# victorkich/ManyTor

Hardware: AMD Instinct MI355X
Metric: env-steps/sec (whole node), 1M parallel 4-DoF arms, random actions (higher is better)
Workload: dtype f32

## Files before the change

### manytor_amd/csrc/engine.hip

```cpp
#include <hip/hip_runtime.h>

#include <algorithm>
#include <cmath>
#include <cstdio>
#include <cstdlib>
#include <cstring>
#include <mutex>
#include <new>
#include <iterator>
#include <string>
#include <utility>
#include <vector>

#include "engine_internal.h"
#include "kernels.h"

using namespace mt;

namespace {
thread_local std::string g_last_error;
}

namespace mt {
int fail(mt_handle h, int code, const std::string& msg) {
// ... 72 lines not shown

struct BlockCap {
  int64_t from, below;
  int blocks;
};
struct DispatchPolicy {
  int64_t step_split4_max = 49152, step_split2_max = 65536;
  int64_t prefetch_other_max = 131072;
  int64_t fused_split4_max = 32768, fused_split2_max = 131072;
  int64_t reset_split_max = 65536;
  int64_t graph_max = 131072;
  int64_t chains_min = 163840, chains_max = 3145728;
  int64_t chain_split4_max = 16384, chain_split2_max = 49152, chain_prefetch_other_max = 131072;
  int64_t flat_from = 393216;
  BlockCap block_caps[3] = {{147456, 229376, 3}, {229376, 458752, 4}, {458752, 589824, 5}};
  int64_t multi_step_max = 262144;
  int multi_step_k = 5;
  bool fold_reset_into_chains = false;
  int max_recurrence_rotations = 12;
  bool rederive_goals_ref4 = true;
  bool rederive_goals_dh7 = false;
  int rederive_goals_chains = 1;
  int64_t rederive_goals_max_envs = 3145728;
  int64_t ld_pad_above = 16384;
  int ld_pad_floats = 256;
};
static const DispatchPolicy kPolicy{};

static int step_blocks_per_cu(const mt_engine* h, int64_t n_launch) {
  if (h->blocks_per_cu_override >= 0) return h->blocks_per_cu_override;
  if (n_launch >= h->n) return 0;
  for (const BlockCap& c : kPolicy.block_caps)
    if (n_launch >= c.from && n_launch < c.below) return c.blocks;
  return 0;
}
static size_t lds_pad_for_blocks(int blocks_per_cu, size_t static_lds) {
  if (blocks_per_cu <= 0) return 0;
  const size_t per_block = (size_t)163840 / (size_t)blocks_per_cu - 1024;
  return per_block > static_lds ? std::min<size_t>(per_block, 65536) - static_lds : 0;
}

int64_t chain_span(const mt_engine* h, int chains) {
  const int64_t per = (h->n + chains - 1) / chains;
  return (per + 255) / 256 * 256;
}

static bool env_int(const char* name, long long* v) {
  const char* e = std::getenv(name);
  if (!e || !*e) return false;
  *v = std::atoll(e);
  return true;
}

static void choose_dispatch(mt_handle h) {
  const mt_config* cfg = &h->cfg;
  const DispatchPolicy& P = kPolicy;
  const int64_t n = cfg->n_envs;
  long long v = 0;
  h->overrides.clear();
  auto seen = [&](const char* name) { h->overrides += (h->overrides.empty() ? "" : ",") + std::string(name) + "=" + std::to_string(v); };

  h->trig = (cfg->flags & MT_FLAG_HW_TRIG) ? 2 : ((cfg->flags & MT_FLAG_DIRECT_TRIG) ? 1 : 0);
  if (cfg->flags & MT_FLAG_ABLATE_LOOP) h->trig = (cfg->flags & MT_FLAG_ABLATE_OBS) ? 4 : 3;
  else if (cfg->flags & MT_FLAG_ABLATE_OBS) h->trig = 5;
  const bool long_route = h->trig == 0 && (cfg->substeps - 1) / 2 > P.max_recurrence_rotations;
  if (long_route) h->trig = 1;
  h->lds_table = (cfg->flags & MT_FLAG_DH_IN_LDS) != 0 && !long_route;
  h->custom_frames = !(h->args.dh.fo == h->D - 2 && h->args.dh.fe == h->D - 1);
  h->static_kind = ((cfg->flags & (MT_FLAG_NO_SPECIALIZE | MT_FLAG_DH_IN_LDS)) || h->custom_frames) ? 0 : match_static(h->args.dh, h->D);

  int forced_lanes = 0, forced_prefetch = -1;
  if (env_int("MT_SPLIT", &v)) {
    forced_lanes = (v == 2 || v == 4) ? (int)v : 1;
    seen("MT_SPLIT");
  }
  if (env_int("MT_PREFETCH", &v)) {
    forced_prefetch = v != 0;
    seen("MT_PREFETCH");
  }
  h->reset_split = n <= P.reset_split_max;
  if (env_int("MT_RESET_SPLIT", &v)) {
    h->reset_split = v != 0;
    seen("MT_RESET_SPLIT");
  }
  h->graph_mode = -1;
  h->graph_max = P.graph_max;
  if (env_int("MT_GRAPH", &v)) {
    h->graph_mode = v != 0 ? 1 : 0;
    seen("MT_GRAPH");
  }
  h->flat_from = P.flat_from;
  if (env_int("MT_FLAT_FROM", &v)) {
    h->flat_from = std::max<long long>(0, v);
    seen("MT_FLAT_FROM");
  }
  h->blocks_per_cu_override = -1;
  if (env_int("MT_BLOCKS_PER_CU", &v)) {
    const int c = (int)std::max<long long>(0, std::min<long long>(8, v));
    h->blocks_per_cu_override = (c == 1 || c == 2) ? 3 : c;
    seen("MT_BLOCKS_PER_CU");
  }
  h->trig_steps = h->static_kind != 0;
  if (env_int("MT_TRIG_TABLE", &v)) {
    h->trig_steps = v != 0 && h->static_kind != 0;
    seen("MT_TRIG_TABLE");
  }
// ... 10 lines not shown
  if (env_int("MT_LAZY_CHAINS", &v)) {
    h->lazy_chains = v != 0;
    seen("MT_LAZY_CHAINS");
  }

  h->multi_k = (n <= P.multi_step_max) ? P.multi_step_k : 1;
  if (env_int("MT_ROLLOUT_K", &v)) {
    h->multi_k = (int)std::max<long long>(1, std::min<long long>(64, v));
    seen("MT_ROLLOUT_K");
  }
  h->defer_reset = true;
  if (env_int("MT_DEFER_RESET", &v)) {
    h->defer_reset = v != 0;
    seen("MT_DEFER_RESET");
  }
  h->defer_reset_chained = P.fold_reset_into_chains;
  if (env_int("MT_DEFER_RESET_CHAINS", &v)) {
    h->defer_reset_chained = v != 0;
    seen("MT_DEFER_RESET_CHAINS");
  }
  h->gather_throttle = true;
  if (env_int("MT_GATHER_THROTTLE", &v)) {
    h->gather_throttle = v != 0;
    seen("MT_GATHER_THROTTLE");
  }
  h->snap_in_rollout = true;
  if (env_int("MT_ROLLOUT_SNAP", &v)) {
    h->snap_in_rollout = v != 0;
    seen("MT_ROLLOUT_SNAP");
  }
  h->rollout_early = true;
  if (env_int("MT_ROLLOUT_EARLY", &v)) {
    h->rollout_early = v != 0;
    seen("MT_ROLLOUT_EARLY");
  }

  h->tape_prefetch = false;
  if (env_int("MT_TAPE_PREFETCH", &v)) {
    h->tape_prefetch = v != 0;
    seen("MT_TAPE_PREFETCH");
  }
  h->tape_nt_loads = false;
  if (env_int("MT_TAPE_NT", &v)) {
    h->tape_nt_loads = v != 0;
    seen("MT_TAPE_NT");
  }

  h->ground_compact = true;
  if (env_int("MT_GROUND_COMPACT", &v)) {
    h->ground_compact = v != 0;
    seen("MT_GROUND_COMPACT");
  }

  h->goals_rederive = h->static_kind == 1 ? P.rederive_goals_ref4 : (h->static_kind == 2 ? P.rederive_goals_dh7 : false);
  h->goals_rederive_chains = P.rederive_goals_chains;
  h->goals_rederive_max_envs = P.rederive_goals_max_envs;
  if (env_int("MT_GOALS_REDERIVE", &v)) {
    h->goals_rederive = v != 0 && h->static_kind != 0;
    h->goals_rederive_chains = mt_engine::kMaxChains;
    h->goals_rederive_max_envs = INT64_MAX;
    seen("MT_GOALS_REDERIVE");
  }

  if (h->custom_frames) h->lds_table = false;
  auto schedule_for = [&](int64_t envs, int64_t split4_max, int64_t split2_max, int64_t prefetch_other_max) {
    mt_engine::Schedule s;
    s.step_lanes = envs <= split4_max ? 4 : (envs <= split2_max ? 2 : 1);
    s.prefetch = h->static_kind == 1 || envs <= prefetch_other_max;
    s.rollout_lanes = envs <= P.fused_split4_max ? 4 : (envs <= P.fused_split2_max ? 2 : 1);
    if (forced_lanes) s.step_lanes = s.rollout_lanes = forced_lanes;
    if (forced_prefetch >= 0) s.prefetch = forced_prefetch != 0;
    if (h->custom_frames) s = mt_engine::Schedule{};
    return s;
  };
  h->sched[mt_engine::kBatch] = schedule_for(n, P.step_split4_max, P.step_split2_max, P.prefetch_other_max);
  h->sched[mt_engine::kChain] =
      h->chains > 1 ? schedule_for(chain_span(h, h->chains), P.chain_split4_max, P.chain_split2_max, P.chain_prefetch_other_max)
                    : h->sched[mt_engine::kBatch];
}

#define MT_DISPATCH_D(D_, FN, ...)   \
  switch (D_) {                      \
    case 2: FN<2>(__VA_ARGS__); break; \
    case 3: FN<3>(__VA_ARGS__); break; \
    case 4: FN<4>(__VA_ARGS__); break; \
    case 5: FN<5>(__VA_ARGS__); break; \
    case 6: FN<6>(__VA_ARGS__); break; \
    case 7: FN<7>(__VA_ARGS__); break; \
    case 8: FN<8>(__VA_ARGS__); break; \
    default: break;                  \
  }

struct StepVariant {
  int trig = 0;
  bool lds = false;
  int lanes = 1;
  int pf = 0;
  bool tt = false;
  bool flat = false;
  bool fresh = false;
  bool codes = false;
  bool gc = false;
  int prev = kPrevLoad;
};
constexpr unsigned variant_key(const StepVariant& v) {
  return (unsigned)v.trig | (unsigned)v.lds << 3 | (unsigned)v.lanes << 4 | (unsigned)(v.pf != 0) << 7 | (unsigned)v.tt << 8 |
         (unsigned)v.flat << 9 | (unsigned)v.fresh << 10 | (unsigned)v.codes << 11 | (unsigned)v.gc << 12 | (unsigned)v.prev << 13;
}

#pragma clang diagnostic push
#pragma clang diagnostic ignored "-Wc++20-designator"
constexpr StepVariant kRuntimeVariants[] = {
    {.trig = 0}, {.trig = 1}, {.trig = 2}, {.trig = 3}, {.trig = 4}, {.trig = 5},
    {.lds = true},
    {.lanes = 2}, {.lanes = 4},
    {.pf = kPrefetch}, {.pf = kPrefetch, .flat = true},
    {.gc = true}, {.pf = kPrefetch, .gc = true}, {.pf = kPrefetch, .flat = true, .gc = true},
// ... 304 lines not shown
  hipLaunchKernelGGL((reset_kernel<D, RANDOM, ONLY_DONE>), grid_for(args.n), dim3(kBlock), lds, h->stream, args,
                     h->cfg.radius);
}
template <int D, bool ONLY_DONE>
void launch_reset_split(mt_handle h, const StepArgs& args) {
  constexpr int L = 4;
  const int64_t per_block = kBlock / L;
  const size_t lds = (size_t)2 * args.K * per_block * sizeof(float);
  hipLaunchKernelGGL((reset_split_kernel<D, ONLY_DONE, L>), dim3((unsigned)((args.n + per_block - 1) / per_block)),
                     dim3(kBlock), lds, h->stream, args, h->cfg.radius);
}
template <int D>
void launch_reset_d(mt_handle h, const StepArgs& args, int mode) {
  if (mode == 0) h->codes_valid = false;
  if (mode != 0 && h->reset_split && args.n == h->n)
    return mode == 1 ? launch_reset_split<D, false>(h, args) : launch_reset_split<D, true>(h, args);
  if (mode == 0)
    launch_reset_k<D, false, false>(h, args);
  else if (mode == 1)
    launch_reset_k<D, true, false>(h, args);
  else
    launch_reset_k<D, true, true>(h, args);
}

template <int D>
void launch_observe_d(mt_handle h) {
  hipLaunchKernelGGL((observe_kernel<D>), grid_for(h->n), dim3(kBlock), 0, h->stream, h->args);
}
template <int D>
void launch_check_done_d(mt_handle h) {
  hipLaunchKernelGGL((check_done_kernel<D>), grid_for(h->n), dim3(kBlock), 0, h->stream, h->args);
}
template <int D>
void launch_joints_d(mt_handle h, float* out) {
  hipLaunchKernelGGL((joints_kernel<D>), grid_for(h->n), dim3(kBlock), 0, h->stream, h->args, out);
}

template <class Tbl, int L, int RPF>
void launch_rollout_split_t(mt_handle h, const StepArgs& a, const RolloutArgs& r) {
  const int64_t per_block = kBlock / L;
  const size_t lds = (size_t)3 * h->K * per_block * sizeof(float) + (ActionTrigTable<Tbl>::value ? kTrigEntries * sizeof(SinCos) : 0);
  if (lds > 65536)
    (void)hipFuncSetAttribute(reinterpret_cast<const void*>(&rollout_split_kernel<Tbl, L, RPF>),
                              hipFuncAttributeMaxDynamicSharedMemorySize, (int)lds);
  hipLaunchKernelGGL((rollout_split_kernel<Tbl, L, RPF>), dim3((unsigned)((a.n + per_block - 1) / per_block)), dim3(kBlock), lds,
                     h->stream, a, r);
}

template <class Tbl, int RPF>
void launch_rollout_t(mt_handle h, const StepArgs& a, int lanes, const RolloutArgs& r) {
  if (lanes == 4) return launch_rollout_split_t<Tbl, 4, RPF>(h, a, r);
  if (lanes == 2) return launch_rollout_split_t<Tbl, 2, RPF>(h, a, r);
  const size_t lds = (size_t)3 * h->K * kBlock * sizeof(float) + (ActionTrigTable<Tbl>::value ? kTrigEntries * sizeof(SinCos) : 0);
  if (lds > 65536)
    (void)hipFuncSetAttribute(reinterpret_cast<const void*>(&rollout_kernel<Tbl, RPF>),
                              hipFuncAttributeMaxDynamicSharedMemorySize, (int)lds);
  hipLaunchKernelGGL((rollout_kernel<Tbl, RPF>), grid_for(a.n), dim3(kBlock), lds, h->stream, a, r);
}

template <int D>
void launch_rollout_d(mt_handle h, const StepArgs& a, int lanes, const RolloutArgs& r) {
  launch_rollout_t<RtTable<D>, 0>(h, a, lanes, r);
}
void launch_rollout(mt_handle h, const StepArgs& a, int lanes, const RolloutArgs& r, bool early = false) {
  h->codes_valid = false;
  h->forget_goals();
  if (h->static_kind == 1) return early ? launch_rollout_t<Ref4Table, kPrefetch>(h, a, lanes, r) : launch_rollout_t<Ref4Table, 0>(h, a, lanes, r);
  if (h->static_kind == 2) return early ? launch_rollout_t<Dh7Table, kPrefetch>(h, a, lanes, r) : launch_rollout_t<Dh7Table, 0>(h, a, lanes, r);
  MT_DISPATCH_D(h->D, launch_rollout_d, h, a, lanes, r);
}

template <class Tbl, bool PREFETCH>
void launch_tape_t(mt_handle h, const StepArgs& a, const TapeArgs& r) {
  const size_t lds = (size_t)3 * h->K * kBlock * sizeof(float);
  if (lds > 65536)
    (void)hipFuncSetAttribute(reinterpret_cast<const void*>(&rollout_tape_kernel<Tbl, PREFETCH>),
                              hipFuncAttributeMaxDynamicSharedMemorySize, (int)lds);
  hipLaunchKernelGGL((rollout_tape_kernel<Tbl, PREFETCH>), grid_for(a.n), dim3(kBlock), lds, h->stream, a, r);
}
template <int D>
void launch_tape_d(mt_handle h, const StepArgs& a, const TapeArgs& r) {
  launch_tape_t<RtTable<D>, false>(h, a, r);
}
bool tape_prefetches(const mt_engine* h) { return h->tape_prefetch && h->static_kind != 0; }
void launch_tape(mt_handle h, const StepArgs& a, const TapeArgs& r) {
  const bool pf = tape_prefetches(h);
  if (h->static_kind == 1) return pf ? launch_tape_t<Ref4Table, true>(h, a, r) : launch_tape_t<Ref4Table, false>(h, a, r);
  if (h->static_kind == 2) return pf ? launch_tape_t<Dh7Table, true>(h, a, r) : launch_tape_t<Dh7Table, false>(h, a, r);
  MT_DISPATCH_D(h->D, launch_tape_d, h, a, r);
}

template <class Tbl>
struct TableTag {
  using type = Tbl;
};
template <class F>
void with_table(const mt_engine* h, F&& f) {
  if (h->static_kind == 1) return f(TableTag<Ref4Table>{});
  if (h->static_kind == 2) return f(TableTag<Dh7Table>{});
  switch (h->D) {
    case 2: return f(TableTag<RtTable<2>>{});
    case 3: return f(TableTag<RtTable<3>>{});
    case 4: return f(TableTag<RtTable<4>>{});
    case 5: return f(TableTag<RtTable<5>>{});
    case 6: return f(TableTag<RtTable<6>>{});
    case 7: return f(TableTag<RtTable<7>>{});
// ... 505 lines not shown
    h->kernel_name += " [mt_rollout: " + std::to_string(h->chains) + " chains of " + std::to_string(chain_span(h, h->chains)) +
                      " envs, " + (c.v.lanes > 1 ? "L=" + std::to_string(c.v.lanes)
                                                 : "pf=" + std::to_string(c.v.pf) + (c.v.flat ? ", flat=1" : "")) +
                      (c.blocks_per_cu > 0 ? ", " + std::to_string(c.blocks_per_cu) + " blocks/CU" : std::string()) + "]";
  }
  if (h->multi_k > 1 && fusable(h)) {
    const int sp = multi_step_lanes(h);
    h->kernel_name += " [mt_rollout: " + std::to_string(h->multi_k) + " steps per launch, " +
                      (sp > 1 ? "rollout_split_kernel L=" + std::to_string(sp) : std::string("rollout_kernel")) + "]";
  }
  return h->kernel_name.c_str();
}

const char* mt_describe_dispatch(mt_handle h) {
  if (!h) return "";
  const DispatchPolicy& P = kPolicy;
  auto num = [](long long v) { return std::to_string(v); };
  auto b = [](bool v) { return std::string(v ? "true" : "false"); };
  const int64_t span = chain_span(h, h->chains);
  const std::string table = table_name(h);
  const StepPlan sb = batch_plan(h), sc = chain_plan(h);
  const bool multi = h->multi_k > 1 && fusable(h);
  const bool graph = h->graph_mode > 0 || (h->graph_mode < 0 && h->n <= h->graph_max);
  const bool rederive_on = h->goals_rederive && !h->goals_exposed && !h->goals_foreign && !h->points_exposed && !h->trace;
  auto rederives = [&](const StepPlan& p) {
    return rederive_on && p.v.lanes == 1 && p.v.pf != 0 && p.v.tt && (&p == &sb ? h->n : span) <= h->goals_rederive_max_envs;
  };
  std::string caps = "[";
  for (const BlockCap& c : P.block_caps) caps += std::string(caps.size() > 1 ? "," : "") + "[" + num(c.from) + "," + num(c.below) + "," + num(c.blocks) + "]";
  caps += "]";
  std::string& d = h->describe;
  d = "{\"n_envs\":" + num(h->n) + ",\"ld\":" + num(h->ld) + ",\"dof\":" + num(h->D) + ",\"targets\":" + num(h->K) +
      ",\"table\":\"" + table + "\",\"trig\":" + num(h->trig) + ",\"lds_table\":" + b(h->lds_table) + ",\"custom_frames\":" + b(h->custom_frames) +
      ",\"step\":{\"lanes_per_env\":" + num(sb.v.lanes) + ",\"prefetch\":" + b(sb.v.pf != 0) +
      ",\"trig_table\":" + b(sb.v.tt) + ",\"flat\":" + b(sb.v.flat) + "}" +
      ",\"chains\":{\"count\":" + num(h->chains) + ",\"span\":" + num(h->chains > 1 ? span : h->n) + ",\"lazy\":" + b(h->lazy_chains) +
      ",\"lanes_per_env\":" + num(sc.v.lanes) + ",\"prefetch\":" + b(sc.v.pf != 0) + ",\"flat\":" + b(sc.v.flat) +
      ",\"blocks_per_cu\":" + num(h->chains > 1 ? sc.blocks_per_cu : 0) + "}" +
      ",\"rollout\":{\"form\":\"" + (multi ? "multi_step" : (h->chains > 1 ? "chained_steps" : (graph ? "graph_replay" : "launch_per_step"))) +
      "\",\"steps_per_launch\":" + num(multi ? h->multi_k : 1) + ",\"graph\":" + b(!multi && graph) +
      ",\"lanes_per_env\":" + num(multi ? multi_step_lanes(h) : (h->chains > 1 ? sc : sb).v.lanes) +
      ",\"chains\":" + num(multi && !h->chains_forced ? 1 : h->chains) +
      ",\"absorbs_reset\":" + b(h->defer_reset && (multi || chained_rollout_absorbs_reset(h))) + ",\"writes_snapshot\":" + b(h->snap_in_rollout && (multi || (h->chains > 1 && !graph && !h->trace))) + "}" +
      ",\"fused\":{\"usable\":" + b(fusable(h)) + ",\"lanes_per_env\":" + num(h->sched[mt_engine::kBatch].rollout_lanes) + "}" +
      ",\"tape\":{\"usable\":" + b(fusable(h)) + ",\"lanes_per_env\":1,\"chains\":1,\"prefetch\":" + b(tape_prefetches(h)) +
      ",\"nt_loads\":" + b(h->tape_nt_loads) + "}" +
      ",\"shoot\":{\"usable\":" + b(fusable(h)) + ",\"envs_per_block\":" + num(kShootEnvs) + ",\"waves_per_block\":" + num(kShootWaves) + "}" +
      ",\"cem\":{\"usable\":" + b(fusable(h)) + ",\"envs_per_block\":" + num(kShootEnvs) + ",\"waves_per_block\":" + num(kShootWaves) +
      ",\"max_candidates\":64}" +
      ",\"mppi\":{\"usable\":" + b(fusable(h)) + ",\"envs_per_block\":" + num(kShootEnvs) + ",\"waves_per_block\":" + num(kShootWaves) +
      ",\"max_candidates\":64,\"max_steps\":" + num(kMppiMaxSteps) + "}" +
      ",\"policy_rollout\":{\"usable\":" + b(fusable(h)) + ",\"lanes_per_env\":1,\"hidden_extents\":[32,64]}" +
      ",\"reset\":{\"lanes_per_env\":" + num(h->reset_split ? 4 : 1) + "}" +
      ",\"ground_compact\":{\"enabled\":" + b(h->ground_compact) + ",\"step\":" + b(sb.v.gc) + ",\"chains\":" + b(sc.v.gc) + "}" +
      ",\"goals\":{\"rederive\":" + b(!multi && !graph && rederives(h->chains > 1 ? sc : sb)) + ",\"enabled\":" + b(h->goals_rederive) +
      ",\"step\":" + b(rederives(sb)) + ",\"chains\":" + b(rederives(sc)) +
      ",\"chains_rederiving\":" + num(rederives(sc) ? std::min(h->chains, h->goals_rederive_chains) : 0) +
      ",\"launches_rederived\":" + num((long long)h->goals_rederived) + "}" +
      ",\"overrides\":\"" + h->overrides + "\"" +
      ",\"policy\":{\"step_split4_max\":" + num(P.step_split4_max) + ",\"step_split2_max\":" + num(P.step_split2_max) +
      ",\"prefetch_other_max\":" + num(P.prefetch_other_max) + ",\"fused_split4_max\":" + num(P.fused_split4_max) +
      ",\"fused_split2_max\":" + num(P.fused_split2_max) + ",\"reset_split_max\":" + num(P.reset_split_max) +
      ",\"graph_max\":" + num(P.graph_max) + ",\"chains_min\":" + num(P.chains_min) + ",\"chains_max\":" + num(P.chains_max) +
      ",\"chain_split4_max\":" + num(P.chain_split4_max) + ",\"chain_split2_max\":" + num(P.chain_split2_max) +
      ",\"chain_prefetch_other_max\":" + num(P.chain_prefetch_other_max) + ",\"flat_from\":" + num(P.flat_from) +
      ",\"block_caps\":" + caps + ",\"multi_step_max\":" + num(P.multi_step_max) + ",\"multi_step_k\":" + num(P.multi_step_k) +
      ",\"max_recurrence_rotations\":" + num(P.max_recurrence_rotations) + ",\"ld_pad_above\":" + num(P.ld_pad_above) +
      ",\"ld_pad_floats\":" + num(P.ld_pad_floats) + ",\"rederive_goals_ref4\":" + b(P.rederive_goals_ref4) +
      ",\"rederive_goals_dh7\":" + b(P.rederive_goals_dh7) + ",\"rederive_goals_chains\":" + num(P.rederive_goals_chains) +
      ",\"rederive_goals_max_envs\":" + num(P.rederive_goals_max_envs) + "}" +
      ",\"arena_bytes\":" + num((long long)h->arena_bytes) + "}";
  return d.c_str();
}

int mt_set_stream(mt_handle h, void* hip_stream) {
  MT_REQUIRE(nullptr, h != nullptr, "handle is NULL");
  MT_ENTER(h);
  MT_HIP(h, hipStreamSynchronize(h->stream));
  h->stream = (hipStream_t)hip_stream;
  return MT_OK;
}

int mt_use_own_stream(mt_handle h) {
  MT_REQUIRE(nullptr, h != nullptr, "handle is NULL");
  MT_ENTER(h);
  MT_HIP(h, hipStreamSynchronize(h->stream));
  h->stream = h->own_stream;
  return MT_OK;
}

int mt_sync(mt_handle h) {
  MT_REQUIRE(nullptr, h != nullptr, "handle is NULL");
  MT_ENTER_KEEP(h);
  MT_HIP(h, hipStreamSynchronize(h->stream));
  if (h->gather_pending) {
    MT_HIP(h, hipStreamSynchronize(h->side_stream));
    MT_HIP(h, hipEventElapsedTime(&h->last_gather_ms, h->ev_g0, h->ev_g1));
    h->gather_pending = false;
    h->snap_free_known[0] = h->snap_free_known[1] = true;
  }
  return MT_OK;
}

int mt_reset(mt_handle h, const float* points, int layout, int is_device) {
  MT_REQUIRE(nullptr, h != nullptr, "handle is NULL");
  MT_REQUIRE(h, points != nullptr, "points is NULL (use mt_reset_random for device-drawn targets)");
  MT_REQUIRE(h, layout == MT_ENV_MAJOR || layout == MT_SOA, "bad layout");
// ... 1996 lines not shown
```

### manytor_amd/csrc/engine_internal.h

```cpp
#pragma once
#include <hip/hip_runtime.h>

#include <cstdlib>
#include <string>
#include <vector>

#include "step_args.h"

struct mt_comm;

struct mt_engine {
  static constexpr int kMaxChains = 4;
  mt_config cfg{};
  int64_t n = 0, ld = 0;
  int D = 0, K = 0;
  hipStream_t own_stream = nullptr;
  hipStream_t stream = nullptr;
  hipEvent_t ev0 = nullptr, ev1 = nullptr;
  hipEvent_t ev1c[kMaxChains] = {nullptr, nullptr, nullptr, nullptr};
  int timer_ends = 0;
  bool timer_with_gather = false;
  struct LapRec {
    uint32_t begin, n_begin, end0, n_end;
  };
// ... 33 lines not shown
    uint64_t seed = 0;
  };
  GoalsRow goals_row[kMaxChains];
  void forget_goals() {
    for (GoalsRow& g : goals_row) g = GoalsRow{};
  }
  void goals_are(GoalsRow::Kind kind, uint64_t seed = 0, uint32_t step = 0) {
    for (GoalsRow& g : goals_row) g = GoalsRow{kind, step, seed};
  }
  bool goals_rederive = true;
  int goals_rederive_chains = kMaxChains;
  int64_t goals_rederive_max_envs = INT64_MAX;
  bool goals_foreign = false;
  uint64_t goals_rederived = 0;
  bool trig_steps = false;
  int static_kind = 0;
  mt_comm* comm = nullptr;
  hipStream_t side_stream = nullptr;
  hipEvent_t ev_snap = nullptr, ev_g0 = nullptr, ev_g1 = nullptr;
  float* snap = nullptr;
  hipEvent_t ev_gdone[2] = {nullptr, nullptr};
  bool snap_free_known[2] = {true, true};
  int snap_next = 0;
  bool gather_throttle = true;
  float* snap_row(int p) const { return snap + (size_t)p * (size_t)n; }
  void* reduce_scratch = nullptr;
  size_t reduce_scratch_bytes = 0;
  bool reset_split = false;
  struct RolloutGraph {
    int T;
    int chains;
    mt::StepArgs args;
    hipGraphExec_t exec[kMaxChains];
  };
  std::vector<RolloutGraph> graphs;
  std::vector<int> graph_seen;
  uint32_t* graph_step0 = nullptr;
  int graph_mode = -1;
  int64_t graph_max = 131072;
  int chains = 1;
  bool chains_forced = false;
  int multi_k = 1;
  bool rollout_early = true;
  bool defer_reset_chained = false;
  bool defer_reset = true;
  bool reset_pending = false;
  uint64_t pend_seed = 0;
  uint32_t pend_episode = 0;
  bool snap_in_rollout = true;
  bool snap_valid = false;
  bool tape_prefetch = false;
  bool tape_nt_loads = false;
  bool ground_compact = true;
  std::string overrides;
  std::string describe;
  hipStream_t chain_streams[kMaxChains] = {nullptr, nullptr, nullptr, nullptr};
  hipEvent_t ev_fork = nullptr, ev_join[kMaxChains] = {nullptr, nullptr, nullptr, nullptr};
  bool forked = false;
  bool lazy_chains = true;
  bool gather_pending = false;
  bool gather_inplace = false;
  float last_gather_ms = 0.f;
  int cu_count = 0;
  std::string err;
  std::string kernel_name;
};

namespace mt {

inline unsigned event_flags(bool timing) {
  static const bool fenced = [] {
    const char* e = std::getenv("MT_EVENT_FENCE");
    return e && *e && std::atoi(e) != 0;
  }();
  return (timing ? 0u : (unsigned)hipEventDisableTiming) | (fenced ? 0u : (unsigned)hipEventDisableSystemFence);
}

int fail(mt_handle h, int code, const std::string& msg);

class DeviceGuard {
 public:
  explicit DeviceGuard(int device) {
    if (hipGetDevice(&prev_) != hipSuccess) prev_ = -1;
    err_ = (prev_ == device) ? hipSuccess : hipSetDevice(device);
    changed_ = (err_ == hipSuccess && prev_ != device);
  }
  ~DeviceGuard() {
    if (changed_ && prev_ >= 0) (void)hipSetDevice(prev_);
  }
  hipError_t error() const { return err_; }

 private:
  int prev_ = -1;
  hipError_t err_ = hipSuccess;
  bool changed_ = false;
};

inline dim3 grid_for(int64_t n) { return dim3((unsigned)((n + kBlock - 1) / kBlock)); }

inline bool snapshot_trusted(mt_engine* h) {
  if (h->stream != h->own_stream) return false;
  hipStreamCaptureStatus st = hipStreamCaptureStatusNone;
  if (hipStreamIsCapturing(h->stream, &st) != hipSuccess) {
    (void)hipGetLastError();
    return false;
  }
// ... 66 lines not shown
```

### manytor_amd/csrc/kernels.h

```cpp
#pragma once
#include <hip/hip_runtime.h>
#include <stdint.h>

#include <type_traits>

#include "mt_math.h"
#include "philox.h"
#include "step_args.h"

namespace mt {

#ifndef MT_NT_STORES
#define MT_NT_STORES 1
#endif
template <typename T>
using global_ptr = __attribute__((address_space(1))) T*;

__device__ __forceinline__ global_ptr<char> uniform_row(const void* row) {
  const uint64_t v = reinterpret_cast<uint64_t>(row);
  const uint32_t lo = __builtin_amdgcn_readfirstlane((uint32_t)v);
  const uint32_t hi = __builtin_amdgcn_readfirstlane((uint32_t)(v >> 32));
  return (global_ptr<char>)(((uint64_t)hi << 32) | lo);
}
#ifndef MT_PLAIN_LANE_OFFSET
// ... 726 lines not shown
  if (um != 0ull) {
    uint32_t base = 0u;
    if ((threadIdx.x & 63u) == 0u) base = atomicAdd(&q.count, (uint32_t)__popcll(um));
    base = (uint32_t)__builtin_amdgcn_readfirstlane((int)base);
    slot = base + __builtin_amdgcn_mbcnt_hi((uint32_t)(um >> 32), __builtin_amdgcn_mbcnt_lo((uint32_t)um, 0u));
  }
  const bool queued = undecided && slot < (uint32_t)kCap;
  if (queued) {
#pragma unroll
    for (int j = 1; j < JN; ++j) {
      float(*f)[kCap] = q.field + 6 * (j - 1);
      f[0][slot] = sF[j];
      f[1][slot] = cF[j];
      f[2][slot] = sA[j];
      f[3][slot] = cA[j];
      f[4][slot] = sd[j];
      f[5][slot] = cd[j];
    }
  }
  if (undecided && !queued) {
    zmin = fminf(zmin, half_route_zmin<Tbl>(t, sF, cF, sd, cd, nf, nf));
#pragma unroll
    for (int j = 1; j < JN; ++j) sd[j] = -sd[j];
    zmin = fminf(zmin, half_route_zmin<Tbl>(t, sA, cA, sd, cd, nf, nb));
  }
  __syncthreads();

  const uint32_t routes = q.count < (uint32_t)kCap ? q.count : (uint32_t)kCap;
  const uint32_t w = (threadIdx.x + 64u * (blockIdx.x & 3u)) & (uint32_t)(kBlock - 1);
  if (w < 2u * routes) {
    const uint32_t r = w >> 1;
    const bool backward = (w & 1u) != 0u;
    float sW[D], cW[D], sdW[D], cdW[D];
#pragma unroll
    for (int j = 0; j < D; ++j) {
      sW[j] = 0.f;
      cW[j] = 1.f;
      sdW[j] = 0.f;
      cdW[j] = 1.f;
    }
#pragma unroll
    for (int j = 1; j < JN; ++j) {
      const float(*f)[kCap] = q.field + 6 * (j - 1);
      sW[j] = backward ? f[2][r] : f[0][r];
      cW[j] = backward ? f[3][r] : f[1][r];
      const float sdj = f[4][r];
      sdW[j] = backward ? -sdj : sdj;
      cdW[j] = f[5][r];
    }
    q.zres[w] = half_route_zmin<Tbl>(t, sW, cW, sdW, cdW, nf, backward ? nb : nf);
  }
  __syncthreads();
  if (queued) zmin = fminf(zmin, fminf(q.zres[2u * slot], q.zres[2u * slot + 1u]));
  return zmin;
}

__device__ __forceinline__ void record_finished(const StepArgs& a, uint32_t i, uint32_t episode, float ret) {
  LaneOffset<true> o4{i * 4u};
  str(a.last_return, o4, ret);
  if (a.ring_slots)
    a.ring[(int64_t)((episode - a.episode0) % a.ring_slots) * a.ld + i] = ret;
}

#ifdef MT_STAMPS
#define MT_STAMP(a, i, slot)                                                                 \
  do {                                                                                       \
    __builtin_amdgcn_sched_barrier(0);                                                       \
    unsigned long long t__;                                                                  \
    asm volatile("s_memtime %0\n\ts_waitcnt lgkmcnt(0)" : "=s"(t__)::"memory");              \
    __builtin_amdgcn_sched_barrier(0);                                                       \
    if ((a).stamps && (threadIdx.x & 63) == 0) (a).stamps[(size_t)((i) >> 6) * 8 + (slot)] = t__; \
  } while (0)
#else
#define MT_STAMP(a, i, slot) \
  do {                       \
  } while (0)
#endif

__device__ __forceinline__ bool unusable_angle(float v) { return (__float_as_uint(v) & 0x7FFFFFFFu) > 0x47000000u; }

template <class Tbl, int TRIG>
constexpr int step_min_waves() { return (TRIG == 0 && Tbl::D >= 6 && Tbl::D <= 7) ? 8 : 1; }

constexpr int kPrefetch = 8;

__device__ __forceinline__ void draw_targets_wave(uint64_t seed, uint64_t env0, uint32_t episode, bool need, int K, float radius,
                                                  float* col0, uint8_t* slots);

enum : int { kPrevLoad = 0, kPrevZero = 1, kPrevDraw = 2 };
template <class Tbl, bool SAMPLE, int TRIG, bool LDS, int PF = 0, bool TT = false, bool FLAT = false, bool FRESH = false,
          bool CODES = false, bool GC = false, int PREV = kPrevLoad>
__global__ __launch_bounds__(kBlock, (PF ? 1 : step_min_waves<Tbl, TRIG>())) void step_kernel(const StepArgs a) {
  constexpr int D = Tbl::D;
  static_assert(PREV == kPrevLoad || CODES, "the previous pose is re-derived by the code-reading kernels (the HBM-bound launches)");
  static_assert(!GC || (TRIG == 0 && !LDS && !FRESH), "the block-cooperative ground test serves the recurrence");
  static_assert(!TT || (SAMPLE && TRIG == 0 && !LDS && ActionTrigTable<Tbl>::value), "the table serves sampled actions of a static table");
  static_assert(!FRESH || TT, "the reset prologue exists for the sampled-action kernels of the static tables");
  static_assert(!CODES || (PF && TT && !FRESH), "codes are read by the prefetch kernels of the static tables");
  extern __shared__ float fresh_stage[];
  __shared__ uint8_t fresh_slots[FRESH ? kBlock / 64 : 1][64];
  __shared__ DhConst sh;
  __shared__ __attribute__((aligned(16))) SinCos trig_lds[TT ? kTrigEntries : 1];
  __shared__ std::conditional_t<GC, GroundQueue<Tbl>, NoGroundQueue> ground_q;
  float4 trig_v;
  if (TT) trig_v = trig_table_load(a.trig_table);
  if constexpr (GC) {
// ... 694 lines not shown
    cell[EPB] = __uint_as_float(c.hi);
  };
  draw_targets_split<L>(seed, env_id, episode, go, K, radius, q, e, put);
  __builtin_amdgcn_wave_barrier();
  if (live && go)
    for (int k = (int)q; k < K; k += L) store_target(a, ld, i, k, staged_code(col + 2 * k * EPB, EPB), radius);
  if (live && q == 0) {
    if (ONLY_DONE && dn == 2) a.done[i] = 0;
    if (go) {
      float s[D], c[D], p[D][3];
#pragma unroll
      for (int j = 0; j < D; ++j) {
        (a.goals + j * ld)[i] = 0.f;
        sincos_deg(a.dh.off_deg[j], s[j], c[j]);
      }
      const RtTableF<D> t{a.dh};
      chain_all<RtTableF<D>>(s, c, t, p);
      float el0[3], e0[3];
      pick_frames<RtTableF<D>>(t, p, el0, e0);
#pragma unroll
      for (int qq = 0; qq < 3; ++qq) (a.ee + qq * ld)[i] = e0[qq];
      if (ONLY_DONE)
        record_finished(a, i, old_episode, old_total);
      else
        a.last_return[i] = old_total;
      a.total_reward[i] = 0.f;
      a.reward[i] = 0;
      a.done[i] = 0;
      a.alive[i] = all_alive_mask(K);
      a.episodes[i] = episode;
    }
  }
  if (lane == 0) a.done_bits[first >> 6] = 0ull;
}

template <int STRIDE>
struct TargetColumn {
  float* col;
  __device__ __forceinline__ float& row(int r) const { return col[r * STRIDE]; }
  __device__ __forceinline__ float& cell(int k, int c) const { return row(3 * k + c); }
  __device__ __forceinline__ float* target(int k) const { return col + 3 * k * STRIDE; }
  __device__ __forceinline__ void get(int k, float& x, float& y, float& z) const { x = target(k)[0], y = target(k)[STRIDE], z = target(k)[2 * STRIDE]; }
  __device__ __forceinline__ void put(int k, float x, float y, float z) const { target(k)[0] = x, target(k)[STRIDE] = y, target(k)[2 * STRIDE] = z; }
  __device__ __forceinline__ void zero(int k) const { put(k, 0.f, 0.f, 0.f); }
};

struct RolloutArgs {
  int32_t T;
  uint32_t step0;
  uint32_t auto_reset;
  float radius;
  uint32_t reset_first, reset_episode, reset_seed_lo, reset_seed_hi;
  float* snap;
};

template <class Tbl, int RPF = 0>
__global__ __launch_bounds__(kBlock) void rollout_kernel(const StepArgs a, const RolloutArgs r) {
  extern __shared__ __attribute__((aligned(16))) float tile[];
  constexpr int D = Tbl::D;
  constexpr bool kTable = ActionTrigTable<Tbl>::value;
  const Tbl t = TableMaker<Tbl>::make(a.dh);
  const SinCos* trig = nullptr;
  float4 trig_v;
  if constexpr (kTable) {
    trig = reinterpret_cast<const SinCos*>(tile + 3 * a.K * kBlock);
    trig_v = trig_table_load(a.trig_table);
    if (!RPF) trig_table_commit(reinterpret_cast<SinCos*>(tile + 3 * a.K * kBlock), trig_v);
  }
  const uint32_t i = blockIdx.x * kBlock + threadIdx.x;
  LaneOffset<true> o4{i * 4u}, o1{i};
  const bool stay = (kTable && RPF) || r.reset_first != 0;
  if (!stay && i >= a.n) return;
  const int64_t ld = a.ld;
  const uint64_t seed = ((uint64_t)a.seed_hi << 32) | a.seed_lo;
  const uint64_t env_id = (uint64_t)(a.env_base + i);
  const TargetColumn<kBlock> tc{tile + threadIdx.x};
  __shared__ uint8_t draw_slots[kBlock / 64][64];

  const uint32_t all_alive = all_alive_mask(a.K);
  const bool fresh = r.reset_first != 0;
  float g[D];
#pragma unroll
  for (int j = 0; j < D; ++j) g[j] = fresh ? 0.f : ldr(a.goals + j * ld, o4);
  uint32_t am = fresh ? all_alive : ldr(a.alive, o4);
  float total = ldr(a.total_reward, o4);
  uint32_t episode = fresh ? r.reset_episode : (r.auto_reset ? ldr(a.episodes, o4) : 0u);
  bool ended = fresh, dirty = fresh;
  float tx[RPF ? RPF : 1][3];
  if (fresh) {
    const bool mine = i < a.n;
    if (mine) str(a.last_return, o4, total);
    total = 0.f;
    const uint32_t lane = threadIdx.x & 63u;
    draw_targets_wave(((uint64_t)r.reset_seed_hi << 32) | r.reset_seed_lo, (uint64_t)(a.env_base + (i - lane)), episode, mine, a.K, r.radius,
                      tile + (threadIdx.x - lane), draw_slots[threadIdx.x >> 6]);
    decode_column(tc.col, a.K, r.radius);
    if (!(kTable && RPF) && !mine) return;
  } else if (RPF) {
#pragma unroll
    for (int k = 0; k < RPF; ++k)
      if (k < a.K) {
#pragma unroll
        for (int q = 0; q < 3; ++q) tx[k][q] = ldr(a.points + (int64_t)(3 * k + q) * ld, o4);
      }
  } else {
    for (int k = 0; k < 3 * a.K; ++k) tc.row(k) = ldr(a.points + (int64_t)k * ld, o4);
  }
  PoseCache<D> pose;
  bool pose_valid = false;

  auto finish_step = [&](const float (&act)[D], const float (&el)[3], const float (&e)[3], float zmin) {
    const bool ground = zmin < 0.f;
    if (a.zmin) str_stream(a.zmin, o4, zmin);

    uint32_t nam = am;
    for (int k = 0; k < a.K; ++k) {
      float x, y, z, dist = 0.f, rr = 0.f, th = 0.f;
      tc.get(k, x, y, z);
      if ((am >> k) & 1u) {
        observe_target(el, x, y, z, dist, rr, th);
        if (within_box(e, x, y, z, a.tol)) nam &= ~(1u << k);
      } else if ((x != 0.f) | (y != 0.f) | (z != 0.f)) {
        tc.zero(k);
        dirty = true;
      }
      float* orow = a.obs + (int64_t)(3 * k) * ld;
      str_stream(orow, o4, dist);
      str_stream(orow + ld, o4, rr);
      str_stream(orow + 2 * ld, o4, th);
    }
    const int32_t rew = ground ? -1 : ((nam != am) ? 1 : 0);
    bool done = (nam == 0u);
    if (a.flags & MT_FLAG_TERMINATE_ON_GROUND) done |= ground;
    total += (float)rew;
    am = nam;
#pragma unroll
    for (int j = 0; j < D; ++j) g[j] = act[j];
#pragma unroll
    for (int q = 0; q < 3; ++q) str_stream(a.ee + q * ld, o4, e[q]);
    str_stream(a.reward, o4, rew);
    str_stream(a.done, o1, (uint8_t)(done ? (r.auto_reset ? 2 : 1) : 0));
    const unsigned long long bits = __ballot(done);
    if ((threadIdx.x & 63) == 0) a.done_bits[i >> 6] = bits;

    if (done && r.auto_reset) {
      record_finished(a, i, episode, total);
      ended = true;
      total = 0.f;
      am = all_alive;
      episode += 1u;
#pragma unroll
      for (int j = 0; j < D; ++j) g[j] = 0.f;
      pose_valid = false;
      draw_targets(seed, env_id, episode, a.K, r.radius, [&](int k, float x, float y, float z) { tc.put(k, x, y, z); });
      dirty = true;
    }
  };

  int s = 0;
  if (RPF) {
    float act[D], el[3], e[3];
    draw_action<D>(seed, env_id, r.step0, act);
    if constexpr (kTable) {
      complete_before_here(act);
      trig_table_commit(reinterpret_cast<SinCos*>(tile + 3 * a.K * kBlock), trig_v);
      if (i >= a.n) return;
    }
    const float zmin = route_kinematics<Tbl, 0, true, kTable>(t, a.S, a.inv_sm1, g, act, el, e, &pose, false, trig,
                                                              (a.flags & kFlagWholeGoals) != 0);
    pose_valid = true;
    if (!fresh) {
#pragma unroll
      for (int k = 0; k < RPF; ++k)
        if (k < a.K) {
#pragma unroll
          for (int q = 0; q < 3; ++q) tc.cell(k, q) = tx[k][q];
        }
      for (int k = 3 * RPF; k < 3 * a.K; ++k) tc.row(k) = ldr(a.points + (int64_t)k * ld, o4);
    }
    finish_step(act, el, e, zmin);
    s = 1;
  }
  for (; s < r.T; ++s) {
    float act[D], el[3], e[3];
    draw_action<D>(seed, env_id, r.step0 + (uint32_t)s, act);
    const float zmin = route_kinematics<Tbl, 0, true, kTable>(t, a.S, a.inv_sm1, g, act, el, e, &pose, pose_valid, trig,
                                                              (a.flags & kFlagWholeGoals) != 0 || s > 0);
    pose_valid = true;
    finish_step(act, el, e, zmin);
  }

#pragma unroll
  for (int j = 0; j < D; ++j) str(a.goals + j * ld, o4, g[j]);
  str(a.alive, o4, am);
  str(a.total_reward, o4, total);
  if (r.snap) str(r.snap, o4, total);
  if (ended) str(a.episodes, o4, episode);
  if (dirty)
    for (int k = 0; k < 3 * a.K; ++k) str(a.points + (int64_t)k * ld, o4, tc.row(k));
}

template <class Tbl, int L, int RPF = 0>
__global__ __launch_bounds__(kBlock) void rollout_split_kernel(const StepArgs a, const RolloutArgs r) {
  static_assert(L == 2 || L == 4, "an env is spread over 2 or 4 lanes");
  extern __shared__ __attribute__((aligned(16))) float tile[];
  constexpr int D = Tbl::D;
  constexpr int EPW = 64 / L;
  constexpr int EPB = kBlock / L;
  constexpr int PFS = (RPF + L - 1) / L;
  constexpr bool kTable = ActionTrigTable<Tbl>::value;
  const Tbl t = TableMaker<Tbl>::make(a.dh);
  const SinCos* trig = nullptr;
  float4 trig_v;
  if constexpr (kTable) {
    trig = reinterpret_cast<const SinCos*>(tile + 3 * a.K * EPB);
    trig_v = trig_table_load(a.trig_table);
    if (!RPF) trig_table_commit(reinterpret_cast<SinCos*>(tile + 3 * a.K * EPB), trig_v);
  }
  const uint32_t lane = threadIdx.x & 63u;
  const uint32_t wave = blockIdx.x * (kBlock / 64) + (threadIdx.x >> 6);
  const uint32_t q = lane / EPW;
  const int64_t first = (int64_t)wave * EPW;
  if (first >= a.n) {
    if constexpr (kTable) {
      if (RPF) trig_table_commit(reinterpret_cast<SinCos*>(tile + 3 * a.K * EPB), trig_v);
    }
    return;
  }
  const uint32_t env = (uint32_t)first + lane % EPW;
  const bool live = env < a.n;
  const uint32_t i = live ? env : (uint32_t)(a.n - 1);
  const int64_t ld = a.ld;
  const uint64_t seed = ((uint64_t)a.seed_hi << 32) | a.seed_lo;
  const uint64_t env_id = (uint64_t)(a.env_base + i);
  const TargetColumn<EPB> tc{tile + (threadIdx.x >> 6) * EPW + lane % EPW};
  const bool backward = (q & 1u) != 0;

  const uint32_t all_alive = all_alive_mask(a.K);
  const bool fresh = r.reset_first != 0;
  float g[D];
// ... 1863 lines not shown
```

Before: 33.24 billion.

## Compact undecided ground-check routes across wave lanes in rollout kernel

Adds a wave-level compaction path to the single-lane rollout kernel. Lanes whose ground-clearance check is still undecided have their interpolated route split into forward and backward halves, and those halves are dealt to idle lanes via ds_bpermute and a small LDS slot table. This targets divergence, where a few lanes walk long substep loops while the rest of the wave sits idle. The cost is extra cross-lane shuffles, wave barriers and register pressure, and the path is enabled by default only for small arms (D<=5) on the default trig route.

```diff
diff --git a/manytor_amd/csrc/engine.hip b/manytor_amd/csrc/engine.hip
--- a/manytor_amd/csrc/engine.hip
+++ b/manytor_amd/csrc/engine.hip
@@ -148,6 +148,11 @@
   return true;
 }
 
+static bool rollout_compacts(const mt_engine* h) {
+  return h->trig == 0 && !h->lds_table && !h->custom_frames && !(h->cfg.flags & MT_FLAG_DEBUG_ZMIN) &&
+         (h->static_kind == 1 || (h->static_kind == 0 && h->D <= 5));
+}
+
 static void choose_dispatch(mt_handle h) {
   const mt_config* cfg = &h->cfg;
   const DispatchPolicy& P = kPolicy;
@@ -264,6 +269,18 @@
     seen("MT_GROUND_COMPACT");
   }
 
+  bool rollout_compact = h->ground_compact;
+  if (env_int("MT_ROLLOUT_COMPACT", &v)) {
+    rollout_compact = rollout_compact && v != 0;
+    seen("MT_ROLLOUT_COMPACT");
+  }
+  h->rollout_compact_cap = 32;
+  if (env_int("MT_ROLLOUT_COMPACT_CAP", &v)) {
+    v = v < 0 ? 0 : (v > 32 ? 32 : v);
+    h->rollout_compact_cap = (uint32_t)v;
+    seen("MT_ROLLOUT_COMPACT_CAP");
+  }
+
   h->goals_rederive = h->static_kind == 1 ? P.rederive_goals_ref4 : (h->static_kind == 2 ? P.rederive_goals_dh7 : false);
   h->goals_rederive_chains = P.rederive_goals_chains;
   h->goals_rederive_max_envs = P.rederive_goals_max_envs;
@@ -275,6 +292,7 @@
   }
 
   if (h->custom_frames) h->lds_table = false;
+  h->rollout_compact = rollout_compact && rollout_compacts(h);
   auto schedule_for = [&](int64_t envs, int64_t split4_max, int64_t split2_max, int64_t prefetch_other_max) {
     mt_engine::Schedule s;
     s.step_lanes = envs <= split4_max ? 4 : (envs <= split2_max ? 2 : 1);
@@ -685,6 +703,17 @@
   if (lanes == 4) return launch_rollout_split_t<Tbl, 4, RPF>(h, a, r);
   if (lanes == 2) return launch_rollout_split_t<Tbl, 2, RPF>(h, a, r);
   const size_t lds = (size_t)3 * h->K * kBlock * sizeof(float) + (ActionTrigTable<Tbl>::value ? kTrigEntries * sizeof(SinCos) : 0);
+  if constexpr (Tbl::D <= 5) {
+    if (h->rollout_compact) {
+      RolloutArgs rc = r;
+      rc.compact_cap = h->rollout_compact_cap;
+      if (lds > 65536)
+        (void)hipFuncSetAttribute(reinterpret_cast<const void*>(&rollout_kernel<Tbl, RPF, true>),
+                                  hipFuncAttributeMaxDynamicSharedMemorySize, (int)lds);
+      hipLaunchKernelGGL((rollout_kernel<Tbl, RPF, true>), grid_for(a.n), dim3(kBlock), lds, h->stream, a, rc);
+      return;
+    }
+  }
   if (lds > 65536)
     (void)hipFuncSetAttribute(reinterpret_cast<const void*>(&rollout_kernel<Tbl, RPF>),
                               hipFuncAttributeMaxDynamicSharedMemorySize, (int)lds);
@@ -1296,7 +1325,8 @@
       ",\"max_candidates\":64,\"max_steps\":" + num(kMppiMaxSteps) + "}" +
       ",\"policy_rollout\":{\"usable\":" + b(fusable(h)) + ",\"lanes_per_env\":1,\"hidden_extents\":[32,64]}" +
       ",\"reset\":{\"lanes_per_env\":" + num(h->reset_split ? 4 : 1) + "}" +
-      ",\"ground_compact\":{\"enabled\":" + b(h->ground_compact) + ",\"step\":" + b(sb.v.gc) + ",\"chains\":" + b(sc.v.gc) + "}" +
+      ",\"ground_compact\":{\"enabled\":" + b(h->ground_compact) + ",\"step\":" + b(sb.v.gc) + ",\"chains\":" + b(sc.v.gc) +
+      ",\"rollout\":" + b(h->rollout_compact) + ",\"rollout_cap\":" + num(h->rollout_compact_cap) + "}" +
       ",\"goals\":{\"rederive\":" + b(!multi && !graph && rederives(h->chains > 1 ? sc : sb)) + ",\"enabled\":" + b(h->goals_rederive) +
       ",\"step\":" + b(rederives(sb)) + ",\"chains\":" + b(rederives(sc)) +
       ",\"chains_rederiving\":" + num(rederives(sc) ? std::min(h->chains, h->goals_rederive_chains) : 0) +
diff --git a/manytor_amd/csrc/engine_internal.h b/manytor_amd/csrc/engine_internal.h
--- a/manytor_amd/csrc/engine_internal.h
+++ b/manytor_amd/csrc/engine_internal.h
@@ -109,6 +109,8 @@
   bool tape_prefetch = false;
   bool tape_nt_loads = false;
   bool ground_compact = true;
+  bool rollout_compact = false;
+  uint32_t rollout_compact_cap = 32;
   std::string overrides;
   std::string describe;
   hipStream_t chain_streams[kMaxChains] = {nullptr, nullptr, nullptr, nullptr};
diff --git a/manytor_amd/csrc/kernels.h b/manytor_amd/csrc/kernels.h
--- a/manytor_amd/csrc/kernels.h
+++ b/manytor_amd/csrc/kernels.h
@@ -802,6 +802,122 @@
   }
   __syncthreads();
   if (queued) zmin = fminf(zmin, fminf(q.zres[2u * slot], q.zres[2u * slot + 1u]));
+  return zmin;
+}
+
+constexpr int kWaveDealRoutes = 32;
+constexpr int kWaveDealSlots = 3 * kWaveDealRoutes;
+__device__ __forceinline__ float lane_pull(uint32_t lane_bytes, float v) {
+  return __int_as_float(__builtin_amdgcn_ds_bpermute((int)lane_bytes, __float_as_int(v)));
+}
+template <class Tbl, bool CACHED, bool TABLE>
+__device__ __forceinline__ float route_kinematics_wave(const Tbl& t, int S, float inv_sm1, const float (&g)[Tbl::D],
+                                                       const float (&act)[Tbl::D], float (&el)[3], float (&e)[3],
+                                                       PoseCache<Tbl::D>* cache, bool cache_valid, const SinCos* trig,
+                                                       bool prev_whole, bool live, uint32_t compact_cap, uint8_t* slots) {
+  constexpr int D = Tbl::D;
+  constexpr int JN = ZJoints<Tbl>::value;
+  static_assert(D <= 5, "the interleaved schedule's end poses; the long arms keep route_kinematics");
+  if (__builtin_expect(__any(live && wide_route<Tbl, TABLE>(g, act, prev_whole)), 0))
+    return route_kinematics_wide<Tbl, CACHED>(t, S, g, act, el, e, cache);
+  const bool use_cache = CACHED && __all(cache_valid);
+
+  float sA[D], cA[D], p[D][3], zo, ze;
+  action_sincos<Tbl, TABLE>(t, act, sA, cA, trig);
+  chain_all<Tbl>(sA, cA, t, p);
+  pick_frames<Tbl>(t, p, el, e);
+  float zmin = fminf(el[2], e[2]);
+  float sF[D], cF[D];
+#pragma unroll
+  for (int j = 0; j < D; ++j) {
+    sF[j] = 0.f;
+    cF[j] = 1.f;
+  }
+  if (use_cache) {
+#pragma unroll
+    for (int j = 1; j < JN; ++j) {
+      sF[j] = cache->s[j];
+      cF[j] = cache->c[j];
+    }
+    zmin = fminf(zmin, cache->zmin);
+  } else {
+    prev_pose_sincos<Tbl, TABLE>(t, g, sF, cF, trig, prev_whole);
+    chain_z<Tbl>(sF, cF, t, zo, ze);
+    zmin = fminf(zmin, fminf(zo, ze));
+  }
+  if (CACHED) {
+#pragma unroll
+    for (int j = 1; j < JN; ++j) {
+      cache->s[j] = sA[j];
+      cache->c[j] = cA[j];
+    }
+    cache->zmin = fminf(el[2], e[2]);
+  }
+
+  const int nf = (S - 1) / 2;
+  const int nb = S - 2 - nf;
+  const bool undecided = live && !(zmin < 0.f);
+  const unsigned long long um = __ballot(undecided);
+  if (um == 0ull || nf == 0) return zmin;
+
+  float st[D], sd[D], cd[D];
+#pragma unroll
+  for (int j = 0; j < D; ++j) st[j] = (act[j] - g[j]) * inv_sm1;
+  sincos_increment<D, JN>(st, sd, cd);
+  sA[0] = 0.f;
+  cA[0] = 1.f;
+
+  const unsigned long long active = __ballot(true);
+  const uint32_t lane = threadIdx.x & 63u;
+  const uint32_t urank = __builtin_amdgcn_mbcnt_hi((uint32_t)(um >> 32), __builtin_amdgcn_mbcnt_lo((uint32_t)um, 0u));
+  uint32_t cap = (uint32_t)__popcll(active) >> 1;
+  cap = cap < (uint32_t)kWaveDealRoutes ? cap : (uint32_t)kWaveDealRoutes;
+  cap = cap < compact_cap ? cap : compact_cap;
+  const uint32_t undecided_lanes = (uint32_t)__popcll(um);
+  const uint32_t routes = undecided_lanes < cap ? undecided_lanes : cap;
+  const bool queued = undecided && urank < routes;
+
+  if (undecided && !queued) {
+    zmin = fminf(zmin, half_route_zmin<Tbl>(t, sF, cF, sd, cd, nf, nf));
+#pragma unroll
+    for (int j = 1; j < JN; ++j) sd[j] = -sd[j];
+    zmin = fminf(zmin, half_route_zmin<Tbl>(t, sA, cA, sd, cd, nf, nb));
+  }
+  if (routes == 0u) return zmin;
+
+  const uint32_t arank = __builtin_amdgcn_mbcnt_hi((uint32_t)(active >> 32), __builtin_amdgcn_mbcnt_lo((uint32_t)active, 0u));
+  const bool worker = arank < 2u * routes;
+  const bool backward = (arank & 1u) != 0u;
+  if (queued) slots[urank] = (uint8_t)lane;
+  if (worker) slots[kWaveDealRoutes + arank] = (uint8_t)lane;
+  __builtin_amdgcn_wave_barrier();
+  const uint32_t from = (worker ? (uint32_t)slots[arank >> 1] : lane) << 2;
+
+  float sW[D], cW[D], sdW[D], cdW[D];
+#pragma unroll
+  for (int j = 0; j < D; ++j) {
+    sW[j] = 0.f;
+    cW[j] = 1.f;
+    sdW[j] = 0.f;
+    cdW[j] = 1.f;
+  }
+#pragma unroll
+  for (int j = 1; j < JN; ++j) {
+    const float sFo = lane_pull(from, sF[j]), cFo = lane_pull(from, cF[j]);
+    const float sAo = lane_pull(from, sA[j]), cAo = lane_pull(from, cA[j]);
+    const float sdo = lane_pull(from, sd[j]);
+    sW[j] = backward ? sAo : sFo;
+    cW[j] = backward ? cAo : cFo;
+    sdW[j] = backward ? -sdo : sdo;
+    cdW[j] = lane_pull(from, cd[j]);
+  }
+  float zhalf = 3.0e38f;
+  if (worker) zhalf = half_route_zmin<Tbl>(t, sW, cW, sdW, cdW, nf, backward ? nb : nf);
+  const uint32_t half0 = (queued ? (uint32_t)slots[kWaveDealRoutes + 2u * urank] : lane) << 2;
+  const uint32_t half1 = (queued ? (uint32_t)slots[kWaveDealRoutes + 2u * urank + 1u] : lane) << 2;
+  __builtin_amdgcn_wave_barrier();
+  const float z0 = lane_pull(half0, zhalf), z1 = lane_pull(half1, zhalf);
+  if (queued) zmin = fminf(zmin, fminf(z0, z1));
   return zmin;
 }
 
@@ -1602,9 +1718,10 @@
   float radius;
   uint32_t reset_first, reset_episode, reset_seed_lo, reset_seed_hi;
   float* snap;
+  uint32_t compact_cap = 32u;
 };
 
-template <class Tbl, int RPF = 0>
+template <class Tbl, int RPF = 0, bool WC = false>
 __global__ __launch_bounds__(kBlock) void rollout_kernel(const StepArgs a, const RolloutArgs r) {
   extern __shared__ __attribute__((aligned(16))) float tile[];
   constexpr int D = Tbl::D;
@@ -1625,7 +1742,7 @@
   const uint64_t seed = ((uint64_t)a.seed_hi << 32) | a.seed_lo;
   const uint64_t env_id = (uint64_t)(a.env_base + i);
   const TargetColumn<kBlock> tc{tile + threadIdx.x};
-  __shared__ uint8_t draw_slots[kBlock / 64][64];
+  __shared__ uint8_t draw_slots[kBlock / 64][WC ? kWaveDealSlots : 64];
 
   const uint32_t all_alive = all_alive_mask(a.K);
   const bool fresh = r.reset_first != 0;
@@ -1659,6 +1776,13 @@
   PoseCache<D> pose;
   bool pose_valid = false;
 
+  auto kinematics = [&](const float (&act)[D], float (&el)[3], float (&e)[3], bool valid, bool prev_whole) __attribute__((always_inline)) {
+    if constexpr (WC)
+      return route_kinematics_wave<Tbl, true, kTable>(t, a.S, a.inv_sm1, g, act, el, e, &pose, valid, trig, prev_whole, true,
+                                                      r.compact_cap, draw_slots[threadIdx.x >> 6]);
+    else
+      return route_kinematics<Tbl, 0, true, kTable>(t, a.S, a.inv_sm1, g, act, el, e, &pose, valid, trig, prev_whole);
+  };
   auto finish_step = [&](const float (&act)[D], const float (&el)[3], const float (&e)[3], float zmin) {
     const bool ground = zmin < 0.f;
     if (a.zmin) str_stream(a.zmin, o4, zmin);
@@ -1716,8 +1840,7 @@
       trig_table_commit(reinterpret_cast<SinCos*>(tile + 3 * a.K * kBlock), trig_v);
       if (i >= a.n) return;
     }
-    const float zmin = route_kinematics<Tbl, 0, true, kTable>(t, a.S, a.inv_sm1, g, act, el, e, &pose, false, trig,
-                                                              (a.flags & kFlagWholeGoals) != 0);
+    const float zmin = kinematics(act, el, e, false, (a.flags & kFlagWholeGoals) != 0);
     pose_valid = true;
     if (!fresh) {
 #pragma unroll
@@ -1734,8 +1857,7 @@
   for (; s < r.T; ++s) {
     float act[D], el[3], e[3];
     draw_action<D>(seed, env_id, r.step0 + (uint32_t)s, act);
-    const float zmin = route_kinematics<Tbl, 0, true, kTable>(t, a.S, a.inv_sm1, g, act, el, e, &pose, pose_valid, trig,
-                                                              (a.flags & kFlagWholeGoals) != 0 || s > 0);
+    const float zmin = kinematics(act, el, e, pose_valid, (a.flags & kFlagWholeGoals) != 0 || s > 0);
     pose_valid = true;
     finish_step(act, el, e, zmin);
   }
```

After: 33.07 billion. About the same (-0.5%).
